# NVIDIAGameWorks/RayTracingDenoiser

Hardware: AMD Instinct MI355X
Metric: Mpixels/s REBLUR_DIFFUSE_SPECULAR @1440p (higher is better)
Workload: dtype f32; 1 GPU; REBLUR_DIFFUSE_SPECULAR 2560x1440, default settings, analytic scene + 1rpp noise, moving camera; parallelism=1 GPU, storage=reference pool formats (fp16 history, R10G10B10A2 normals)

## Files before the change

raytracingdenoiser_amd/csrc/hip/kernels_reblur_history.hip:

```cpp
#include "passes.h"
#include "reblur_device.h"

namespace nrdhip {

constexpr int TILE_X = 32;
constexpr int TILE_Y = 8;

static const char* CheckSupportedHistory(const ReblurCB& c) {
    if (c.gRectOrigin.x != 0 || c.gRectOrigin.y != 0)
        return "internal error: a pass was handed a non-zero rectOrigin";
    if (c.gOrthoMode != 0.0f)
        return "REBLUR: orthographic projection is not supported (SURVEY.md section 8c)";
    return nullptr;
}

static_assert(TILE_X == 32 && TILE_Y == 8, "planes.h LoadBlockTileBytes: a workgroup covers two 16x16 tiles of one tile row");

namespace hf {
constexpr int BORDER = 2;
constexpr int BUF_X = TILE_X + 2 * BORDER;
constexpr int BUF_Y = TILE_Y + 2 * BORDER;
constexpr int BUF_STRIDE = BUF_X + 1;

constexpr int TAPS = 20;
constexpr uint64_t PackTaps(bool rows) {
    uint64_t packed = 0;
    int k = 0;
    for (int j = -2; j <= 2; j++)
        for (int i = -2; i <= 2; i++) {
            if ((i == 0 && j == 0) || ((i < 0 ? -i : i) + (j < 0 ? -j : j) == 4))
                continue;
            packed |= uint64_t((rows ? j : i) + 2) << (3 * k++);
        }
    return packed;
}
constexpr uint64_t TAP_I = PackTaps(false), TAP_J = PackTaps(true);
}

namespace hf {
constexpr int TAP_BATCH = 2;
static_assert(TAP_BATCH > 0 && TAPS % TAP_BATCH == 0, "hf::TAP_BATCH: a divisor of 20");
}

struct HfPlanes {
    Plane tiles, normalRoughness, data1, viewZ, inDiff, inSpec, inDiffFast, inSpecFast, outDiff, outSpec, outDiffFast, outSpecFast;
    Plane inDiffSh, inSpecSh, outDiffSh, outSpecSh;
    NormalRoughnessGuide decodedNR;
};

struct HfPixel {
    int px, py, tx, ty;
    float viewZ, roughness, materialID, frustumSize;
    float3 N, Nv, Xv;
    float2 pixelUv;
};

template <bool IS_SPEC, bool DIFF, bool SPEC, bool PERF, int KIND, bool SH>
NRD_D typename ReblurSignal<KIND>::type HistoryFixSignal(const ReblurCB& c, const HfPlanes& P, const HfPixel& s, typename ReblurSignal<KIND>::type sig, float frameNum, float strideBase,
    const Plane& gIn_Signal, const Plane& gIn_Fast, const Plane& gOut_Fast, const float* s_Luma, float4& sh, const Plane& gIn_Sh) {
    typedef ReblurSignal<KIND> Sig;
    typedef typename Sig::type S;
    const int rw = c.gRectSizeMinusOne.x, rh = c.gRectSizeMinusOne.y;
    const float smc = GetSpecMagicCurve(s.roughness);

    float stride = strideBase * (frameNum < c.gHistoryFixFrameNum ? 1.0f : 0.0f);
    if (IS_SPEC)
        stride *= Lerp(0.5f, 1.0f, smc);
    stride = floorf(stride);

    if (stride != 0.0f) {
        const int stridei = (int)(stride + 0.5f);
        const float nonLinearAccumSpeed = Rcp(1.0f + frameNum);
        const float r = IS_SPEC ? s.roughness : 1.0f;
        const float2 rectSizeInv = ToF2(c.gRectSizeInv);
        const float4 hitDistParams = ToF4(c.gHitDistParams);

        float normalWeightParam = GetNormalWeightParam(nonLinearAccumSpeed, c.gLobeAngleFraction, r);
        float2 geometryWeightParams = GetGeometryWeightParams(c.gPlaneDistSensitivity, s.frustumSize, s.Xv, s.Nv);
        float2 relaxedRoughnessWeightParams = GetRelaxedRoughnessWeightParams(s.roughness * s.roughness, Sqrt(c.gRoughnessFraction));

        float hitDistScale = GetHitDistanceNormalization(s.viewZ, hitDistParams, r);
        float hitDist = ExtractHitDist(sig) * hitDistScale;
        float hitDistFactor = GetHitDistFactor(hitDist, s.frustumSize);
        float2 hitDistanceWeightParams = GetHitDistanceWeightParams(hitDistFactor, nonLinearAccumSpeed, r);

        float sumw = 1.0f + frameNum;
        if (PERF)
            sumw = 1.0f + Rcp(1.0f + c.gMaxAccumulatedFrameNum) - nonLinearAccumSpeed;
        sig = sig * sumw;
        if (SH)
            sh = F4(sh.x * sumw, sh.y * sumw, sh.z * sumw, IS_SPEC ? sh.w : sh.w * sumw);

        const float minMaterial = IS_SPEC ? c.gSpecMinMaterial : c.gDiffMinMaterial;
        const bool compareMaterials = minMaterial < 3.0f;

        const float rcpFrustumSize = Rcp(s.frustumSize);
        const float hitDistEdgeBase = LinearStep(0.03f, 0.05f, s.roughness);
        const float hitDistEdge = 0.2f + hitDistEdgeBase;
        const float hitDistRcpRange = Rcp((0.05f + hitDistEdgeBase) - hitDistEdge);

        struct Tap {
            float4 normalViewZ;
            uint32_t roughnessWord;
            float2 data1;
            S smp;
            float4 sh;
        };
        auto reconstruct = [&](auto materials) {
            constexpr bool MATERIALS = decltype(materials)::value;
            auto requestTap = [&](int i, int j) {
                const int sx = ClampI(s.px + i * stridei, 0, rw), sy = ClampI(s.py + j * stridei, 0, rh);
                Tap t;
                const uint32_t offset = TexelOffset(P.decodedNR.nz, sx, sy, 16u, true);
                t.normalViewZ = *(const float4*)(P.decodedNR.nz.ptr + offset);
                t.roughnessWord = 0u;
                if (IS_SPEC || MATERIALS)
                    t.roughnessWord = *(const uint32_t*)(P.decodedNR.word.ptr + (offset >> 2));
                t.data1 = F2(0.0f, 0.0f);
                if (!PERF)
                    t.data1 = LoadData1<DIFF, SPEC>(P.data1, sx, sy);
                t.smp = Sig::Load(gIn_Signal, sx, sy);
                t.sh = F4(0.0f);
                if (SH)
                    t.sh = LoadRGBA16F(gIn_Sh, sx, sy);
                return t;
            };
            auto addTap = [&](const Tap& t, int i, int j) {
                float2 uv = s.pixelUv + F2(float(i), float(j)) * stride * rectSizeInv;

                float zs = t.normalViewZ.w;
                float4 Ns = F4(t.normalViewZ.x, t.normalViewZ.y, t.normalViewZ.z, DecodedRoughness(t.roughnessWord));

                float angle = AcosApprox(Dot(Xyz(Ns), s.N));
                float3 Xvs = ReconstructViewPosition(uv, ToF4(c.gFrustum), zs, NRD_ORTHO_MODE(c));

                float w = IsInScreenNearest(uv);
                w *= ComputeWeight(Dot(s.Nv, Xvs), geometryWeightParams.x, geometryWeightParams.y);
                if (MATERIALS)
                    w *= CompareMaterials(s.materialID, DecodedMaterialID(t.roughnessWord), minMaterial) ? 1.0f : 0.0f;
                w *= ComputeExponentialWeight(angle, normalWeightParam, 0.0f);
                if (IS_SPEC)
                    w *= ComputeExponentialWeight(Ns.w * Ns.w, relaxedRoughnessWeightParams.x, relaxedRoughnessWeightParams.y);

                if (!PERF)
                    w *= 1.0f + (IS_SPEC ? t.data1.y : t.data1.x);

                S smp = Select(w == 0.0f, Sig::Zero(), t.smp);

                float hs = ExtractHitDist(smp) * hitDistScale;
                float hsFactor = Sat(hs * rcpFrustumSize);
                w *= ComputeExponentialWeight(hsFactor, hitDistanceWeightParams.x, hitDistanceWeightParams.y);

                if (IS_SPEC) {
                    float d = Div(Abs(hitDist - hs), Max(hitDist, hs) + 0.001f);
                    w *= SmoothStep01(Sat((d - hitDistEdge) * hitDistRcpRange));
                }

                sumw += w;
                sig = Mad(smp, w, sig);
                if (SH) {
                    float4 tsh = Select(w == 0.0f, F4(0.0f), t.sh);
                    sh = F4(sh.x + tsh.x * w, sh.y + tsh.y * w, sh.z + tsh.z * w, IS_SPEC ? sh.w : sh.w + tsh.w * w);
                }
            };

#pragma unroll 1
            for (int first = 0; first < hf::TAPS; first += hf::TAP_BATCH) {
                Tap taps[hf::TAP_BATCH];
#pragma unroll
                for (int n = 0; n < hf::TAP_BATCH; n++)
                    taps[n] = requestTap(int((hf::TAP_I >> (3 * (first + n))) & 7u) - 2, int((hf::TAP_J >> (3 * (first + n))) & 7u) - 2);
#pragma unroll
                for (int n = 0; n < hf::TAP_BATCH; n++)
                    addTap(taps[n], int((hf::TAP_I >> (3 * (first + n))) & 7u) - 2, int((hf::TAP_J >> (3 * (first + n))) & 7u) - 2);
            }
        };
        if (compareMaterials)
            reconstruct(std::true_type());
        else
            reconstruct(std::false_type());

        sumw = PositiveRcp(sumw);
        sig = sig * sumw;
        if (SH)
            sh = F4(sh.x * sumw, sh.y * sumw, sh.z * sumw, IS_SPEC ? sh.w : sh.w * sumw);
    }

    float center = s_Luma[(s.ty + hf::BORDER) * hf::BUF_STRIDE + s.tx + hf::BORDER];
    float m1 = center, m2 = center * center;

    float f = Sat(Div(frameNum, c.gHistoryFixFrameNum + NRD_EPS));
    if (IS_SPEC)
        f = Lerp(1.0f, f, smc);
    center = Lerp(GetLuma(sig), center, f);
    Sig::StoreFast(gOut_Fast, s.px, s.py, center);

#pragma unroll
    for (int j = 0; j <= 4; j++) {
#pragma unroll
        for (int i = 0; i <= 4; i++) {
            if (i == 2 && j == 2)
                continue;
            float d = s_Luma[(s.ty + j) * hf::BUF_STRIDE + s.tx + i];
            m1 += d;
            m2 += d * d;
        }
    }

    float luma = GetLuma(sig);

    if (KIND == SIGNAL_RADIANCE && c.gAntiFirefly != 0.0f) {
        float am1 = 0.0f, am2 = 0.0f;
        const int R = PERF ? 3 : REBLUR_ANTI_FIREFLY_FILTER_RADIUS;
        for (int j = -R; j <= R; j++)
            for (int i = -R; i <= R; i++) {
                if (abs(i) <= 1 && abs(j) <= 1)
                    continue;
                float d = LoadR16F(gIn_Fast, ClampI(s.px + i, 0, rw), ClampI(s.py + j, 0, rh));
                am1 += d;
                am2 += d * d;
            }
        float invNorm = Rcp(float((R * 2 + 1) * (R * 2 + 1) - 3 * 3));
        am1 *= invNorm;
        am2 *= invNorm;
        float sigma = Sqrt(Abs(am2 - am1 * am1)) * REBLUR_ANTI_FIREFLY_SIGMA_SCALE;
        luma = Clamp(luma, am1 - sigma, am1 + sigma);
    }

    m1 = m1 * (1.0f / 25.0f);
    m2 = m2 * (1.0f / 25.0f);
    float sigma = Sqrt(Abs(m2 - m1 * m1)) * (KIND != SIGNAL_RADIANCE ? REBLUR_COLOR_CLAMPING_SIGMA_SCALE_OCCLUSION : REBLUR_COLOR_CLAMPING_SIGMA_SCALE);
    float lumaClamped = Clamp(luma, m1 - sigma, m1 + sigma);
    luma = Lerp(lumaClamped, luma, Rcp(1.0f + (c.gMaxFastAccumulatedFrameNum < c.gMaxAccumulatedFrameNum ? 1.0f : 0.0f) * frameNum * 2.0f));

    if (SH) {
        float k = GetLumaScale(Length(Xyz(sh)), luma);
        sh = F4(sh.x * k, sh.y * k, sh.z * k, sh.w);
    }
    return ChangeLuma(sig, luma);
}

template <bool DIFF, bool SPEC, bool PERF, int KIND, bool SH>
__global__ __launch_bounds__(TILE_X* TILE_Y, SH ? 0 : NRD_WAVES_REBLUR_HF - (PERF ? 1 : 0)) void ReblurHistoryFixKernel(ReblurCB c, HfPlanes P, RowRange rr) {
    typedef ReblurSignal<KIND> Sig;
    typedef typename Sig::type S;
    __shared__ float s_DiffLuma[DIFF ? hf::BUF_Y * hf::BUF_STRIDE : 1];
    __shared__ float s_SpecLuma[SPEC ? hf::BUF_Y * hf::BUF_STRIDE : 1];

    const int tx = threadIdx.x % TILE_X, ty = threadIdx.x / TILE_X;
    const int blockY = BlockTileY(rr);
    const int tileX = BlockTileXRotated(rr, blockY);
    const int px = tileX * TILE_X + tx, py = blockY * TILE_Y + ty;
    const int rw = c.gRectSizeMinusOne.x, rh = c.gRectSizeMinusOne.y;

    const uint32_t tileBytes = LoadBlockTileBytes(P.tiles, tileX, blockY);
    if (!TileBytesHaveGeometry<2>(tileBytes))
        return;
    const int qx = min(px, rw), qy = min(max(py, 0), rh);
    const bool preSky = TileByteIsSky(tileBytes, tx >> 4);
    float preMaterialID, preViewZ;
    const float4 preNormalAndRoughness = LoadDecodedNormalRoughness(P.decodedNR, qx, qy, preMaterialID, preViewZ);
    const float2 preData1 = LoadData1<DIFF, SPEC>(P.data1, qx, qy);
    S preDiff = Sig::Zero(), preSpec = Sig::Zero();
    if (DIFF)
        preDiff = Sig::Load(P.inDiff, qx, qy);
    if (SPEC)
        preSpec = Sig::Load(P.inSpec, qx, qy);
    {
        const int baseX = tileX * TILE_X - hf::BORDER, baseY = blockY * TILE_Y - hf::BORDER;
        for (int i = threadIdx.x; i < hf::BUF_X * hf::BUF_Y; i += TILE_X * TILE_Y) {
            int lx = i % hf::BUF_X, ly = i / hf::BUF_X;
            int gx = ClampI(baseX + lx, 0, rw), gy = ClampI(baseY + ly, 0, rh);
            if (DIFF)
                s_DiffLuma[ly * hf::BUF_STRIDE + lx] = Sig::LoadFast(P.inDiffFast, gx, gy);
            if (SPEC)
                s_SpecLuma[ly * hf::BUF_STRIDE + lx] = Sig::LoadFast(P.inSpecFast, gx, gy);
        }
    }
    __syncthreads();

    if (px > rw || py > rh || py < rr.rowBegin || py >= rr.rowEnd)
        return;
    if (preSky)
        return;
    HfPixel s;
    s.viewZ = preViewZ;
    if (s.viewZ > c.gDenoisingRange)
        return;

    s.px = px, s.py = py, s.tx = tx, s.ty = ty;
    s.materialID = preMaterialID;
    float4 normalAndRoughness = preNormalAndRoughness;
    s.N = Xyz(normalAndRoughness);
    s.roughness = normalAndRoughness.w;
    s.frustumSize = GetFrustumSize(c.gMinRectDimMulUnproject, NRD_ORTHO_MODE(c), s.viewZ);
    s.pixelUv = F2(float(px) + 0.5f, float(py) + 0.5f) * ToF2(c.gRectSizeInv);
    s.Xv = ReconstructViewPosition(s.pixelUv, ToF4(c.gFrustum), s.viewZ, NRD_ORTHO_MODE(c));
    s.Nv = RotateVectorInverse(c.gViewToWorld, s.N);
    float2 frameNum = preData1;
    float2 stride = F2(Div(c.gHistoryFixBasePixelStride, 2.0f + frameNum.x), Div(c.gHistoryFixBasePixelStride, 2.0f + frameNum.y));

    if (DIFF) {
        float4 diffSh = F4(0.0f);
        if (SH)
            diffSh = LoadRGBA16F(P.inDiffSh, px, py);
        S diff = HistoryFixSignal<false, DIFF, SPEC, PERF, KIND, SH>(c, P, s, preDiff, frameNum.x, stride.x, P.inDiff, P.inDiffFast, P.outDiffFast, s_DiffLuma, diffSh, P.inDiffSh);
        Sig::Store(P.outDiff, px, py, diff);
        if (SH)
            StoreRGBA16F(P.outDiffSh, px, py, diffSh);
    }
    if (SPEC) {
        float4 specSh = F4(0.0f);
        if (SH)
            specSh = LoadRGBA16F(P.inSpecSh, px, py);
        S spec = HistoryFixSignal<true, DIFF, SPEC, PERF, KIND, SH>(c, P, s, preSpec, frameNum.y, stride.y, P.inSpec, P.inSpecFast, P.outSpecFast, s_SpecLuma, specSh, P.inSpecSh);
        Sig::Store(P.outSpec, px, py, spec);
        if (SH)
            StoreRGBA16F(P.outSpecSh, px, py, specSh);
    }
}

template <bool DIFF, bool SPEC, bool PERF, int KIND, bool SH>
static const char* LaunchHistoryFix(const PassArgs& a) {
    const ReblurCB& c = *(const ReblurCB*)a.constants;
    if (const char* err = CheckSupportedHistory(c))
        return err;
    HfPlanes P = {};
    uint32_t k = 0;
    P.tiles = a.planes[k++];
    P.normalRoughness = a.planes[k++];
    if (const char* err = MakeNormalRoughnessGuide(a, P.decodedNR))
        return err;
    P.data1 = a.planes[k++];
    P.viewZ = a.planes[k++];
    if (DIFF) P.inDiff = a.planes[k++];
    if (SPEC) P.inSpec = a.planes[k++];
    if (DIFF) P.inDiffFast = a.planes[k++];
    if (SPEC) P.inSpecFast = a.planes[k++];
    if (DIFF && SH) P.inDiffSh = a.planes[k++];
    if (SPEC && SH) P.inSpecSh = a.planes[k++];
    if (DIFF) P.outDiff = a.planes[k++];
    if (SPEC) P.outSpec = a.planes[k++];
    if (DIFF) P.outDiffFast = a.planes[k++];
    if (SPEC) P.outSpecFast = a.planes[k++];
    if (DIFF && SH) P.outDiffSh = a.planes[k++];
    if (SPEC && SH) P.outSpecSh = a.planes[k++];
    if (k != a.planesNum)
        return "REBLUR history fix: unexpected resource count";
    RowGrid g = GridForRows(c.gRectSizeMinusOne.x + 1, c.gRectSizeMinusOne.y + 1, TILE_X, TILE_Y, a.rowBegin, a.rowEnd);
    LaunchPass(a, (ReblurHistoryFixKernel<DIFF, SPEC, PERF, KIND, SH>), g.grid, dim3(TILE_X * TILE_Y), c, P, MakeRowRange(g));
    return nullptr;
}

namespace ts {
constexpr int BORDER = 1;
constexpr int BUF_X = TILE_X + 2 * BORDER;
constexpr int BUF_Y = TILE_Y + 2 * BORDER;
constexpr int BUF_STRIDE = BUF_X + 1;
}

struct TsPlanes {
    Plane tiles, normalRoughness, viewZ, data1, data2, inDiff, inSpec, historyDiffLuma, historySpecLuma, inSpecHitDistForTracking, mv, outInternalData, outDiff, outSpec, outDiffLuma,
        outSpecLuma;
    Plane inDiffSh, inSpecSh, outDiffSh, outSpecSh;
    NormalRoughnessGuide decodedNR;
    Plane baseColorMetalness;
};

template <bool PERF>
NRD_D void LumaStats(const ReblurCB& c, const float* s_Luma, int tx, int ty, float& luma, float& m1, float& sigma) {
    luma = s_Luma[(ty + ts::BORDER) * ts::BUF_STRIDE + tx + ts::BORDER];
    float M1 = luma, M2 = luma * luma, mn = NRD_INF, mx = -NRD_INF;
#pragma unroll
    for (int j = 0; j <= 2; j++) {
#pragma unroll
        for (int i = 0; i <= 2; i++) {
            if (i == 1 && j == 1)
                continue;
            float d = s_Luma[(ty + j) * ts::BUF_STRIDE + tx + i];
            M1 += d;
            M2 += d * d;
            mn = Min(mn, d);
            mx = Max(mx, d);
        }
    }
    M1 = M1 * (1.0f / 9.0f);
    M2 = M2 * (1.0f / 9.0f);
    m1 = M1;
    sigma = Sqrt(Abs(M2 - M1 * M1));
    if (!PERF && c.gMaxBlurRadius != 0.0f)
        luma = Clamp(luma, mn, mx);
}

template <bool DIFF, bool SPEC, bool PERF, bool SH, int KIND, bool MVMOD>
__global__ __launch_bounds__(TILE_X* TILE_Y, NRD_WAVES_REBLUR_TS) void ReblurTemporalStabilizationKernel(ReblurCB c, TsPlanes P, RowRange rr) {
    typedef ReblurSignal<KIND> Sig;
    typedef typename Sig::type S;
    __shared__ float s_DiffLuma[DIFF ? ts::BUF_Y * ts::BUF_STRIDE : 1];
    __shared__ float s_SpecLuma[SPEC ? ts::BUF_Y * ts::BUF_STRIDE : 1];

    const int tx = threadIdx.x % TILE_X, ty = threadIdx.x / TILE_X;
    const int blockY = BlockTileY(rr);
    const int px = BlockTileX(rr) * TILE_X + tx, py = blockY * TILE_Y + ty;
    const int rw = c.gRectSizeMinusOne.x, rh = c.gRectSizeMinusOne.y;

    const uint32_t tileBytes = LoadBlockTileBytes(P.tiles, BlockTileX(rr), blockY);
    if (!TileBytesHaveGeometry<2>(tileBytes))
        return;
    const int qx = min(px, rw), qy = min(max(py, 0), rh);
    const bool preSky = TileByteIsSky(tileBytes, tx >> 4);
    const float preViewZ = LoadR32F(P.viewZ, qx, qy);
    const float4 preMv = LoadRGBA16F(P.mv, qx, qy);
    float preMaterialID;
    const float4 preNormalAndRoughness = LoadDecodedNormalRoughness(P.decodedNR, qx, qy, preMaterialID);
    const float2 preData1 = LoadData1<DIFF, SPEC>(P.data1, qx, qy);
    const uint32_t preData2 = SPEC ? LoadR32U(P.data2, qx, qy) : LoadR8U(P.data2, qx, qy);
    S preDiff = Sig::Zero(), preSpec = Sig::Zero();
    if (DIFF)
        preDiff = Sig::Load(P.inDiff, qx, qy);
    if (SPEC)
        preSpec = Sig::Load(P.inSpec, qx, qy);
    {
        const int baseX = BlockTileX(rr) * TILE_X - ts::BORDER, baseY = blockY * TILE_Y - ts::BORDER;
        for (int i = threadIdx.x; i < ts::BUF_X * ts::BUF_Y; i += TILE_X * TILE_Y) {
            int lx = i % ts::BUF_X, ly = i / ts::BUF_X;
            int gx = ClampI(baseX + lx, 0, rw), gy = ClampI(baseY + ly, 0, rh);
            if (DIFF)
                s_DiffLuma[ly * ts::BUF_STRIDE + lx] = GetLuma(Sig::Load(P.inDiff, gx, gy));
            if (SPEC)
                s_SpecLuma[ly * ts::BUF_STRIDE + lx] = GetLuma(Sig::Load(P.inSpec, gx, gy));
        }
    }
    __syncthreads();
// ... 251 lines not shown
```

raytracingdenoiser_amd/csrc/hip/planes.h:

```cpp
#pragma once

#include <hip/hip_fp16.h>
#include <hip/hip_runtime.h>

#include <cstdint>
#include <type_traits>

namespace nrdhip {

struct Plane {
    uint8_t* ptr;
    uint32_t pitch;
    int32_t w, h;
};

#define NRD_D __device__ __forceinline__

NRD_D void ShareLayout(Plane& p, const Plane& ref) {
    p.pitch = ref.pitch;
    p.w = ref.w;
    p.h = ref.h;
}
NRD_D void ShareSize(Plane& p, const Plane& ref) {
    p.w = ref.w;
// ... 33 lines not shown
#define NRD_DIV_15(k) DivSmallIntByConst(k, 15.0f, 0.06666667014360428f)
#define NRD_DIV_3(k) DivSmallIntByConst(k, 3.0f, 0.3333333432674408f)

#ifndef NRD_LDS_WHOLE_TEXEL
#define NRD_LDS_WHOLE_TEXEL(v) asm("" : "+v"(v.x), "+v"(v.y), "+v"(v.z), "+v"(v.w))
#endif
NRD_D float4 LdsFloat4(const float4* p) {
    float4 v = *p;
    NRD_LDS_WHOLE_TEXEL(v);
    return v;
}

NRD_D float HalfBitsToFloat(uint16_t h) { return __half2float(__ushort_as_half(h)); }
#ifndef NRD_OPAQUE_CVT_F16
#define NRD_OPAQUE_CVT_F16(h, f) asm("v_cvt_f16_f32 %0, %1" : "=v"(h) : "v"(f))
#endif
NRD_D uint16_t FloatToHalfBits(float f) {
    uint32_t h;
    NRD_OPAQUE_CVT_F16(h, f);
    return (uint16_t)h;
}

NRD_D float LoadR32F(const Plane& p, int x, int y) { return *TexelPtr<const float>(p, x, y); }
NRD_D void StoreR32F(const Plane& p, int x, int y, float v) { *TexelPtr<float>(p, x, y) = v; }
NRD_D uint32_t LoadR32U(const Plane& p, int x, int y) { return *TexelPtr<const uint32_t>(p, x, y); }
NRD_D void StoreR32U(const Plane& p, int x, int y, uint32_t v) { *TexelPtr<uint32_t>(p, x, y) = v; }
NRD_D uint32_t LoadR16U(const Plane& p, int x, int y) { return *TexelPtr<const uint16_t>(p, x, y); }
NRD_D void StoreR16U(const Plane& p, int x, int y, uint32_t v) { *TexelPtr<uint16_t>(p, x, y) = (uint16_t)v; }
NRD_D uint32_t LoadR8U(const Plane& p, int x, int y) { return *TexelPtr<const uint8_t>(p, x, y); }
NRD_D void StoreR8U(const Plane& p, int x, int y, uint32_t v) { *TexelPtr<uint8_t>(p, x, y) = (uint8_t)v; }

template <int N, int BPT = 1>
NRD_D uint32_t LoadTileBytesUniform(const Plane& tiles, int tileX0, int tileY) {
    static_assert((N == 1 || N == 2 || N == 4) && (BPT == 1 || BPT == 2) && N * BPT <= 4, "the tiles under a workgroup lie in one aligned dword");
    const int cx = min(tileX0, tiles.w - 1), cy = min(tileY, tiles.h - 1);
    uint32_t bytes = 0;
#if defined(__HIP_DEVICE_COMPILE__)
    const uint32_t offset = (uint32_t)__builtin_amdgcn_readfirstlane((int)(__umul24((uint32_t)cy, tiles.pitch) + (((uint32_t)cx * BPT) & ~3u)));
    typedef const uint32_t __attribute__((address_space(4))) ConstDword;
    const uint32_t raw = *(ConstDword*)(uintptr_t)(tiles.ptr + offset) >> ((((uint32_t)cx * BPT) & 3u) * 8u);
    for (int t = 0; t < N; t++)
        bytes |= ((raw >> (8 * BPT * t)) & 0xFFu) << (8 * t);
#else
    for (int t = 0; t < N; t++)
        bytes |= (cx + t < tiles.w ? (uint32_t)tiles.ptr[(uint32_t)cy * tiles.pitch + (uint32_t)(cx + t) * BPT] : 0xFFu) << (8 * t);
#endif
    uint32_t outside = (tileX0 >= tiles.w || tileY >= tiles.h) ? 0xFFFFFFFFu : 0u;
    for (int t = 1; t < N; t++)
        outside |= tileX0 + t >= tiles.w ? 0xFFu << (8 * t) : 0u;
    return (bytes | outside) & (N == 4 ? 0xFFFFFFFFu : (1u << (8 * (N & 3))) - 1u);
}
template <int N>
NRD_D bool TileBytesHaveGeometry(uint32_t bytes) {
    bool any = false;
    for (int t = 0; t < N; t++)
        any |= ((bytes >> (8 * t)) & 0xFFu) == 0u;
    return any;
}
NRD_D bool TileByteIsSky(uint32_t bytes, int t) { return ((bytes >> (8 * t)) & 0xFFu) != 0u; }
NRD_D uint32_t LoadBlockTileBytes(const Plane& tiles, int blockX, int blockY) { return LoadTileBytesUniform<2>(tiles, blockX * 2, blockY >> 1); }

constexpr int TILE_FLAG_GROUP = 64;
NRD_D bool AnyTileFlagUniform(const Plane& flags, int firstTile, int row) {
    const int count = min(flags.w - firstTile, TILE_FLAG_GROUP);
    uint32_t any = 0;
#if defined(__HIP_DEVICE_COMPILE__)
    typedef uint32_t Dwords __attribute__((ext_vector_type(TILE_FLAG_GROUP / 4)));
    typedef const Dwords __attribute__((address_space(4))) ConstDwords;
    const uint32_t offset = (uint32_t)__builtin_amdgcn_readfirstlane((int)(__umul24((uint32_t)row, flags.pitch) + (uint32_t)firstTile));
    const Dwords v = *(ConstDwords*)(uintptr_t)(flags.ptr + offset);
#pragma unroll
    for (int i = 0; i < TILE_FLAG_GROUP / 4; i++) {
        const int n = count - 4 * i;
        any |= n >= 4 ? v[i] : (n > 0 ? v[i] & ((1u << (8 * n)) - 1u) : 0u);
    }
#else
    for (int k = 0; k < count; k++)
        any |= flags.ptr[(uint32_t)row * flags.pitch + (uint32_t)(firstTile + k)];
#endif
    return any != 0u;
}
NRD_D bool TileFlagUniform(const Plane& flags, int tile, int row) { return LoadTileBytesUniform<1>(flags, tile, row) != 0u; }

NRD_D float LoadR16F(const Plane& p, int x, int y) { return HalfBitsToFloat(*TexelPtr<const uint16_t>(p, x, y)); }
NRD_D void StoreR16F(const Plane& p, int x, int y, float v) { *TexelPtr<uint16_t>(p, x, y) = FloatToHalfBits(v); }

NRD_D float4 LoadRGBA16F(const Plane& p, int x, int y) {
    uint2 raw = *TexelPtr<const uint2>(p, x, y);
    float4 r;
    r.x = HalfBitsToFloat((uint16_t)(raw.x & 0xFFFFu));
    r.y = HalfBitsToFloat((uint16_t)(raw.x >> 16));
    r.z = HalfBitsToFloat((uint16_t)(raw.y & 0xFFFFu));
    r.w = HalfBitsToFloat((uint16_t)(raw.y >> 16));
    return r;
}
#ifndef NRD_OPAQUE_CVT_PK_F16
#define NRD_OPAQUE_CVT_PK_F16(r, a, b) asm("v_cvt_pk_f16_f32 %0, %1, %2" : "=v"(r) : "v"(a), "v"(b))
#endif
NRD_D uint32_t FloatsToHalf2Bits(float lo, float hi) {
    uint32_t r;
    NRD_OPAQUE_CVT_PK_F16(r, lo, hi);
    return r;
}
NRD_D void StoreRGBA16F(const Plane& p, int x, int y, float4 v) {
    uint2 raw;
    raw.x = FloatsToHalf2Bits(v.x, v.y);
    raw.y = FloatsToHalf2Bits(v.z, v.w);
    *TexelPtr<uint2>(p, x, y) = raw;
}

#ifndef NRD_NT_STORE_PIXELS
#define NRD_NT_STORE_PIXELS 6000000u
#endif
template <bool NT>
NRD_D void StoreRGBA16FHinted(const Plane& p, int x, int y, float4 v) {
    if constexpr (NT) {
        typedef uint32_t V2 __attribute__((ext_vector_type(2)));
        V2 raw;
        raw.x = FloatsToHalf2Bits(v.x, v.y);
        raw.y = FloatsToHalf2Bits(v.z, v.w);
        __builtin_nontemporal_store(raw, (V2*)TexelPtr<uint2>(p, x, y));
    } else {
        StoreRGBA16F(p, x, y, v);
    }
}

NRD_D float4 LoadRGBA32F(const Plane& p, int x, int y) { return *TexelPtr<const float4>(p, x, y); }
NRD_D void StoreRGBA32F(const Plane& p, int x, int y, float4 v) { *TexelPtr<float4>(p, x, y) = v; }

struct Rgb32Texel {
    float x, y, z;
};
static_assert(sizeof(Rgb32Texel) == 12 && alignof(Rgb32Texel) == 4, "RGB32_SFLOAT texels are three packed dwords");
NRD_D float3 LoadXyz32F(const Plane& p, int x, int y, uint32_t bytesPerTexel) {
    const Rgb32Texel v = *(const Rgb32Texel*)(p.ptr + TexelOffset(p, x, y, bytesPerTexel, true));
    return make_float3(v.x, v.y, v.z);
}
NRD_D float3 LoadRGB32F(const Plane& p, int x, int y) { return LoadXyz32F(p, x, y, 12u); }
NRD_D void StoreRGB32F(const Plane& p, int x, int y, float3 v) { *TexelPtr<Rgb32Texel>(p, x, y) = Rgb32Texel{v.x, v.y, v.z}; }

NRD_D float Saturate(float x) { return fminf(fmaxf(x, 0.0f), 1.0f); }
NRD_D uint32_t ToUnorm(float x, float maxValue) { return (uint32_t)floorf(Saturate(x) * maxValue + 0.5f); }

NRD_D float LoadR8Unorm(const Plane& p, int x, int y) { return NRD_DIV_255(float(*TexelPtr<const uint8_t>(p, x, y))); }
NRD_D void StoreR8Unorm(const Plane& p, int x, int y, float v) { *TexelPtr<uint8_t>(p, x, y) = (uint8_t)ToUnorm(v, 255.0f); }

NRD_D float LoadR16Unorm(const Plane& p, int x, int y) { return NRD_DIV_65535(float(*TexelPtr<const uint16_t>(p, x, y))); }
NRD_D void StoreR16Unorm(const Plane& p, int x, int y, float v) { *TexelPtr<uint16_t>(p, x, y) = (uint16_t)ToUnorm(v, 65535.0f); }

NRD_D float FromSnorm16(uint32_t bits16) { return fmaxf(NRD_DIV_32767(float((int32_t)(int16_t)bits16)), -1.0f); }
NRD_D uint32_t ToSnorm16(float x) {
    float c = fminf(fmaxf(x, -1.0f), 1.0f) * 32767.0f;
    int32_t i = c >= 0.0f ? (int32_t)floorf(c + 0.5f) : -(int32_t)floorf(-c + 0.5f);
    return (uint32_t)i & 0xFFFFu;
}
NRD_D float4 LoadRGBA16Snorm(const Plane& p, int x, int y) {
    uint2 raw = *TexelPtr<const uint2>(p, x, y);
    return make_float4(FromSnorm16(raw.x & 0xFFFFu), FromSnorm16(raw.x >> 16), FromSnorm16(raw.y & 0xFFFFu), FromSnorm16(raw.y >> 16));
}
NRD_D void StoreRGBA16Snorm(const Plane& p, int x, int y, float4 v) {
    uint2 raw;
    raw.x = ToSnorm16(v.x) | (ToSnorm16(v.y) << 16);
    raw.y = ToSnorm16(v.z) | (ToSnorm16(v.w) << 16);
    *TexelPtr<uint2>(p, x, y) = raw;
}

// ... 38 lines not shown
```

Baseline: 5401 Mpixels/s.

## Redistribute history-fix reconstruction taps cooperatively across the workgroup

Adds a cooperative path to the REBLUR history-fix kernel. When only a few pixels in a tile have young history and need the 20-tap reconstruction, their per-pixel parameters are stored in LDS and the (pixel, tap) jobs are spread over all threads, so sparse divergent waves no longer run the full tap loop serially. A cost heuristic (and an env override) decides between the cooperative path and the original per-pixel loop. The cost is extra LDS, extra barriers, ballots and recomputation of per-pixel state, and the path is compiled only when SH is off.

New measurement: 5426 Mpixels/s, median of 6. About the same (+0.5%).

```diff
diff --git a/raytracingdenoiser_amd/csrc/hip/kernels_reblur_history.hip b/raytracingdenoiser_amd/csrc/hip/kernels_reblur_history.hip
--- a/raytracingdenoiser_amd/csrc/hip/kernels_reblur_history.hip
+++ b/raytracingdenoiser_amd/csrc/hip/kernels_reblur_history.hip
@@ -1,5 +1,7 @@
 #include "passes.h"
 #include "reblur_device.h"
+
+#include <cstdio>
 
 namespace nrdhip {
 
@@ -42,6 +44,12 @@
 static_assert(TAP_BATCH > 0 && TAPS % TAP_BATCH == 0, "hf::TAP_BATCH: a divisor of 20");
 }
 
+namespace hf {
+constexpr int MAX_PAIRS = 32;
+constexpr int MAX_JOBS = MAX_PAIRS * TAPS;
+constexpr int KAPPA_NUM = 3, KAPPA_DEN = 2;
+}
+
 struct HfPlanes {
     Plane tiles, normalRoughness, data1, viewZ, inDiff, inSpec, inDiffFast, inSpecFast, outDiff, outSpec, outDiffFast, outSpecFast;
     Plane inDiffSh, inSpecSh, outDiffSh, outSpecSh;
@@ -49,44 +57,191 @@
 };
 
 struct HfPixel {
-    int px, py, tx, ty;
+    int px, py, x0, y0;
     float viewZ, roughness, materialID, frustumSize;
     float3 N, Nv, Xv;
     float2 pixelUv;
 };
 
+struct alignas(16) HfTapParams {
+    int px, py;
+    float stride, materialID;
+    float3 N;
+    float normalWeightParam;
+    float3 Nv;
+    float hitDistScale;
+    float2 pixelUv, geometryWeightParams;
+    float2 relaxedRoughnessWeightParams, hitDistanceWeightParams;
+    float hitDist, rcpFrustumSize, hitDistEdge, hitDistRcpRange;
+};
+static_assert(sizeof(HfTapParams) == 96, "hf::MAX_PAIRS: the LDS budget counts 96 bytes per pair");
+
+template <typename S>
+struct HfTap {
+    float4 normalViewZ;
+    uint32_t roughnessWord;
+    float2 data1;
+    S smp;
+    float4 sh;
+};
+
+template <bool IS_SPEC>
+NRD_D float HistoryFixStride(const ReblurCB& c, float frameNum, float strideBase, float smc) {
+    float stride = strideBase * (frameNum < c.gHistoryFixFrameNum ? 1.0f : 0.0f);
+    if (IS_SPEC)
+        stride *= Lerp(0.5f, 1.0f, smc);
+    return floorf(stride);
+}
+
+template <bool IS_SPEC, typename S>
+NRD_D HfTapParams MakeHfTapParams(const ReblurCB& c, const HfPixel& s, S sig, float frameNum, float stride) {
+    const float nonLinearAccumSpeed = Rcp(1.0f + frameNum);
+    const float r = IS_SPEC ? s.roughness : 1.0f;
+    const float4 hitDistParams = ToF4(c.gHitDistParams);
+
+    HfTapParams t;
+    t.px = s.px, t.py = s.py;
+    t.stride = stride;
+    t.materialID = s.materialID;
+    t.N = s.N, t.Nv = s.Nv;
+    t.pixelUv = s.pixelUv;
+    t.normalWeightParam = GetNormalWeightParam(nonLinearAccumSpeed, c.gLobeAngleFraction, r);
+    t.geometryWeightParams = GetGeometryWeightParams(c.gPlaneDistSensitivity, s.frustumSize, s.Xv, s.Nv);
+    t.relaxedRoughnessWeightParams = F2(0.0f, 0.0f);
+    if (IS_SPEC)
+        t.relaxedRoughnessWeightParams = GetRelaxedRoughnessWeightParams(s.roughness * s.roughness, Sqrt(c.gRoughnessFraction));
+
+    t.hitDistScale = GetHitDistanceNormalization(s.viewZ, hitDistParams, r);
+    t.hitDist = ExtractHitDist(sig) * t.hitDistScale;
+    float hitDistFactor = GetHitDistFactor(t.hitDist, s.frustumSize);
+    t.hitDistanceWeightParams = GetHitDistanceWeightParams(hitDistFactor, nonLinearAccumSpeed, r);
+
+    t.rcpFrustumSize = Rcp(s.frustumSize);
+    t.hitDistEdge = 0.0f, t.hitDistRcpRange = 0.0f;
+    if (IS_SPEC) {
+        const float hitDistEdgeBase = LinearStep(0.03f, 0.05f, s.roughness);
+        t.hitDistEdge = 0.2f + hitDistEdgeBase;
+        t.hitDistRcpRange = Rcp((0.05f + hitDistEdgeBase) - t.hitDistEdge);
+    }
+    return t;
+}
+
+template <bool PERF>
+NRD_D float HfOwnWeight(const ReblurCB& c, float frameNum) {
+    float sumw = 1.0f + frameNum;
+    if (PERF)
+        sumw = 1.0f + Rcp(1.0f + c.gMaxAccumulatedFrameNum) - Rcp(1.0f + frameNum);
+    return sumw;
+}
+
+template <bool IS_SPEC, bool DIFF, bool SPEC, bool PERF, int KIND, bool SH, bool MATERIALS>
+NRD_D HfTap<typename ReblurSignal<KIND>::type> HfRequestTap(const ReblurCB& c, const HfPlanes& P, const HfTapParams& p, const Plane& gIn_Signal, const Plane& gIn_Sh, int i, int j) {
+    typedef ReblurSignal<KIND> Sig;
+    const int rw = c.gRectSizeMinusOne.x, rh = c.gRectSizeMinusOne.y;
+    const int stridei = (int)(p.stride + 0.5f);
+    const int sx = ClampI(p.px + i * stridei, 0, rw), sy = ClampI(p.py + j * stridei, 0, rh);
+    HfTap<typename Sig::type> t;
+    const uint32_t offset = TexelOffset(P.decodedNR.nz, sx, sy, 16u, true);
+    t.normalViewZ = *(const float4*)(P.decodedNR.nz.ptr + offset);
+    t.roughnessWord = 0u;
+    if (IS_SPEC || MATERIALS)
+        t.roughnessWord = *(const uint32_t*)(P.decodedNR.word.ptr + (offset >> 2));
+    t.data1 = F2(0.0f, 0.0f);
+    if (!PERF)
+        t.data1 = LoadData1<DIFF, SPEC>(P.data1, sx, sy);
+    t.smp = Sig::Load(gIn_Signal, sx, sy);
+    t.sh = F4(0.0f);
+    if (SH)
+        t.sh = LoadRGBA16F(gIn_Sh, sx, sy);
+    return t;
+}
+template <bool IS_SPEC, bool PERF, int KIND, bool MATERIALS>
+NRD_D float HfTapWeight(const ReblurCB& c, const HfTapParams& p, float minMaterial, const HfTap<typename ReblurSignal<KIND>::type>& t, int i, int j,
+    typename ReblurSignal<KIND>::type& smp) {
+    const float2 rectSizeInv = ToF2(c.gRectSizeInv);
+    float2 uv = p.pixelUv + F2(float(i), float(j)) * p.stride * rectSizeInv;
+
+    float zs = t.normalViewZ.w;
+    float4 Ns = F4(t.normalViewZ.x, t.normalViewZ.y, t.normalViewZ.z, DecodedRoughness(t.roughnessWord));
+
+    float angle = AcosApprox(Dot(Xyz(Ns), p.N));
+    float3 Xvs = ReconstructViewPosition(uv, ToF4(c.gFrustum), zs, NRD_ORTHO_MODE(c));
+
+    float w = IsInScreenNearest(uv);
+    w *= ComputeWeight(Dot(p.Nv, Xvs), p.geometryWeightParams.x, p.geometryWeightParams.y);
+    if (MATERIALS)
+        w *= CompareMaterials(p.materialID, DecodedMaterialID(t.roughnessWord), minMaterial) ? 1.0f : 0.0f;
+    w *= ComputeExponentialWeight(angle, p.normalWeightParam, 0.0f);
+    if (IS_SPEC)
+        w *= ComputeExponentialWeight(Ns.w * Ns.w, p.relaxedRoughnessWeightParams.x, p.relaxedRoughnessWeightParams.y);
+
+    if (!PERF)
+        w *= 1.0f + (IS_SPEC ? t.data1.y : t.data1.x);
+
+    smp = Select(w == 0.0f, ReblurSignal<KIND>::Zero(), t.smp);
+
+    float hs = ExtractHitDist(smp) * p.hitDistScale;
+    float hsFactor = Sat(hs * p.rcpFrustumSize);
+    w *= ComputeExponentialWeight(hsFactor, p.hitDistanceWeightParams.x, p.hitDistanceWeightParams.y);
+
+    if (IS_SPEC) {
+        float d = Div(Abs(p.hitDist - hs), Max(p.hitDist, hs) + 0.001f);
+        w *= SmoothStep01(Sat((d - p.hitDistEdge) * p.hitDistRcpRange));
+    }
+    return w;
+}
+
+template <bool IS_SPEC, bool DIFF, bool SPEC, bool PERF, int KIND, bool MATERIALS>
+NRD_D void HfCoopTap(const ReblurCB& c, const HfPlanes& P, const Plane& gIn_Signal, float minMaterial, const HfTapParams* s_Rec, int rec, int k, float* s_TapW,
+    typename ReblurSignal<KIND>::type* s_TapSmp, int slot) {
+    const HfTapParams p = s_Rec[rec];
+    const int i = int((hf::TAP_I >> (3 * k)) & 7u) - 2, j = int((hf::TAP_J >> (3 * k)) & 7u) - 2;
+    const auto t = HfRequestTap<IS_SPEC, DIFF, SPEC, PERF, KIND, false, MATERIALS>(c, P, p, gIn_Signal, gIn_Signal, i, j);
+    typename ReblurSignal<KIND>::type smp;
+    const float w = HfTapWeight<IS_SPEC, PERF, KIND, MATERIALS>(c, p, minMaterial, t, i, j, smp);
+    s_TapW[slot] = w;
+    s_TapSmp[slot] = smp;
+}
+template <bool IS_SPEC, bool DIFF, bool SPEC, bool PERF, int KIND>
+NRD_D void HfCoopTaps(const ReblurCB& c, const HfPlanes& P, const Plane& gIn_Signal, const HfTapParams* s_Rec, int firstRec, int count, int first, float* s_TapW,
+    typename ReblurSignal<KIND>::type* s_TapSmp) {
+    const float minMaterial = IS_SPEC ? c.gSpecMinMaterial : c.gDiffMinMaterial;
+    const bool compareMaterials = minMaterial < 3.0f;
+    for (int n = first; n < count * hf::TAPS; n += TILE_X * TILE_Y) {
+        const int pair = n / hf::TAPS, k = n - pair * hf::TAPS;
+        if (compareMaterials)
+            HfCoopTap<IS_SPEC, DIFF, SPEC, PERF, KIND, true>(c, P, gIn_Signal, minMaterial, s_Rec, firstRec + pair, k, s_TapW, s_TapSmp, firstRec * hf::TAPS + n);
+        else
+            HfCoopTap<IS_SPEC, DIFF, SPEC, PERF, KIND, false>(c, P, gIn_Signal, minMaterial, s_Rec, firstRec + pair, k, s_TapW, s_TapSmp, firstRec * hf::TAPS + n);
+    }
+}
+template <bool PERF, typename S>
+NRD_D S HfCoopSum(const ReblurCB& c, S sig, float frameNum, const float* s_TapW, const S* s_TapSmp, int rec) {
+    float sumw = HfOwnWeight<PERF>(c, frameNum);
+    sig = sig * sumw;
+#pragma unroll 4
+    for (int k = 0; k < hf::TAPS; k++) {
+        const float w = s_TapW[rec * hf::TAPS + k];
+        const S smp = s_TapSmp[rec * hf::TAPS + k];
+        sumw += w;
+        sig = Mad(smp, w, sig);
+    }
+    sumw = PositiveRcp(sumw);
+    return sig * sumw;
+}
+
 template <bool IS_SPEC, bool DIFF, bool SPEC, bool PERF, int KIND, bool SH>
-NRD_D typename ReblurSignal<KIND>::type HistoryFixSignal(const ReblurCB& c, const HfPlanes& P, const HfPixel& s, typename ReblurSignal<KIND>::type sig, float frameNum, float strideBase,
-    const Plane& gIn_Signal, const Plane& gIn_Fast, const Plane& gOut_Fast, const float* s_Luma, float4& sh, const Plane& gIn_Sh) {
+NRD_D typename ReblurSignal<KIND>::type HistoryFixSignal(const ReblurCB& c, const HfPlanes& P, const HfPixel& s, typename ReblurSignal<KIND>::type sig, float frameNum, float stride,
+    bool reconstructed, const Plane& gIn_Signal, const Plane& gIn_Fast, const Plane& gOut_Fast, const float* s_Luma, float4& sh, const Plane& gIn_Sh) {
     typedef ReblurSignal<KIND> Sig;
     typedef typename Sig::type S;
     const int rw = c.gRectSizeMinusOne.x, rh = c.gRectSizeMinusOne.y;
     const float smc = GetSpecMagicCurve(s.roughness);
 
-    float stride = strideBase * (frameNum < c.gHistoryFixFrameNum ? 1.0f : 0.0f);
-    if (IS_SPEC)
-        stride *= Lerp(0.5f, 1.0f, smc);
-    stride = floorf(stride);
-
-    if (stride != 0.0f) {
-        const int stridei = (int)(stride + 0.5f);
-        const float nonLinearAccumSpeed = Rcp(1.0f + frameNum);
-        const float r = IS_SPEC ? s.roughness : 1.0f;
-        const float2 rectSizeInv = ToF2(c.gRectSizeInv);
-        const float4 hitDistParams = ToF4(c.gHitDistParams);
-
-        float normalWeightParam = GetNormalWeightParam(nonLinearAccumSpeed, c.gLobeAngleFraction, r);
-        float2 geometryWeightParams = GetGeometryWeightParams(c.gPlaneDistSensitivity, s.frustumSize, s.Xv, s.Nv);
-        float2 relaxedRoughnessWeightParams = GetRelaxedRoughnessWeightParams(s.roughness * s.roughness, Sqrt(c.gRoughnessFraction));
-
-        float hitDistScale = GetHitDistanceNormalization(s.viewZ, hitDistParams, r);
-        float hitDist = ExtractHitDist(sig) * hitDistScale;
-        float hitDistFactor = GetHitDistFactor(hitDist, s.frustumSize);
-        float2 hitDistanceWeightParams = GetHitDistanceWeightParams(hitDistFactor, nonLinearAccumSpeed, r);
-
-        float sumw = 1.0f + frameNum;
-        if (PERF)
-            sumw = 1.0f + Rcp(1.0f + c.gMaxAccumulatedFrameNum) - nonLinearAccumSpeed;
+    if (stride != 0.0f && !reconstructed) {
+        const HfTapParams p = MakeHfTapParams<IS_SPEC>(c, s, sig, frameNum, stride);
+
+        float sumw = HfOwnWeight<PERF>(c, frameNum);
         sig = sig * sumw;
         if (SH)
             sh = F4(sh.x * sumw, sh.y * sumw, sh.z * sumw, IS_SPEC ? sh.w : sh.w * sumw);
@@ -94,68 +249,11 @@
         const float minMaterial = IS_SPEC ? c.gSpecMinMaterial : c.gDiffMinMaterial;
         const bool compareMaterials = minMaterial < 3.0f;
 
-        const float rcpFrustumSize = Rcp(s.frustumSize);
-        const float hitDistEdgeBase = LinearStep(0.03f, 0.05f, s.roughness);
-        const float hitDistEdge = 0.2f + hitDistEdgeBase;
-        const float hitDistRcpRange = Rcp((0.05f + hitDistEdgeBase) - hitDistEdge);
-
-        struct Tap {
-            float4 normalViewZ;
-            uint32_t roughnessWord;
-            float2 data1;
-            S smp;
-            float4 sh;
-        };
         auto reconstruct = [&](auto materials) {
             constexpr bool MATERIALS = decltype(materials)::value;
-            auto requestTap = [&](int i, int j) {
-                const int sx = ClampI(s.px + i * stridei, 0, rw), sy = ClampI(s.py + j * stridei, 0, rh);
-                Tap t;
-                const uint32_t offset = TexelOffset(P.decodedNR.nz, sx, sy, 16u, true);
-                t.normalViewZ = *(const float4*)(P.decodedNR.nz.ptr + offset);
-                t.roughnessWord = 0u;
-                if (IS_SPEC || MATERIALS)
-                    t.roughnessWord = *(const uint32_t*)(P.decodedNR.word.ptr + (offset >> 2));
-                t.data1 = F2(0.0f, 0.0f);
-                if (!PERF)
-                    t.data1 = LoadData1<DIFF, SPEC>(P.data1, sx, sy);
-                t.smp = Sig::Load(gIn_Signal, sx, sy);
-                t.sh = F4(0.0f);
-                if (SH)
-                    t.sh = LoadRGBA16F(gIn_Sh, sx, sy);
-                return t;
-            };
-            auto addTap = [&](const Tap& t, int i, int j) {
-                float2 uv = s.pixelUv + F2(float(i), float(j)) * stride * rectSizeInv;
-
-                float zs = t.normalViewZ.w;
-                float4 Ns = F4(t.normalViewZ.x, t.normalViewZ.y, t.normalViewZ.z, DecodedRoughness(t.roughnessWord));
-
-                float angle = AcosApprox(Dot(Xyz(Ns), s.N));
-                float3 Xvs = ReconstructViewPosition(uv, ToF4(c.gFrustum), zs, NRD_ORTHO_MODE(c));
-
-                float w = IsInScreenNearest(uv);
-                w *= ComputeWeight(Dot(s.Nv, Xvs), geometryWeightParams.x, geometryWeightParams.y);
-                if (MATERIALS)
-                    w *= CompareMaterials(s.materialID, DecodedMaterialID(t.roughnessWord), minMaterial) ? 1.0f : 0.0f;
-                w *= ComputeExponentialWeight(angle, normalWeightParam, 0.0f);
-                if (IS_SPEC)
-                    w *= ComputeExponentialWeight(Ns.w * Ns.w, relaxedRoughnessWeightParams.x, relaxedRoughnessWeightParams.y);
-
-                if (!PERF)
-                    w *= 1.0f + (IS_SPEC ? t.data1.y : t.data1.x);
-
-                S smp = Select(w == 0.0f, Sig::Zero(), t.smp);
-
-                float hs = ExtractHitDist(smp) * hitDistScale;
-                float hsFactor = Sat(hs * rcpFrustumSize);
-                w *= ComputeExponentialWeight(hsFactor, hitDistanceWeightParams.x, hitDistanceWeightParams.y);
-
-                if (IS_SPEC) {
-                    float d = Div(Abs(hitDist - hs), Max(hitDist, hs) + 0.001f);
-                    w *= SmoothStep01(Sat((d - hitDistEdge) * hitDistRcpRange));
-                }
-
+            auto addTap = [&](const HfTap<S>& t, int i, int j) {
+                S smp;
+                const float w = HfTapWeight<IS_SPEC, PERF, KIND, MATERIALS>(c, p, minMaterial, t, i, j, smp);
                 sumw += w;
                 sig = Mad(smp, w, sig);
                 if (SH) {
@@ -166,10 +264,11 @@
 
 #pragma unroll 1
             for (int first = 0; first < hf::TAPS; first += hf::TAP_BATCH) {
-                Tap taps[hf::TAP_BATCH];
+                HfTap<S> taps[hf::TAP_BATCH];
 #pragma unroll
                 for (int n = 0; n < hf::TAP_BATCH; n++)
-                    taps[n] = requestTap(int((hf::TAP_I >> (3 * (first + n))) & 7u) - 2, int((hf::TAP_J >> (3 * (first + n))) & 7u) - 2);
+                    taps[n] = HfRequestTap<IS_SPEC, DIFF, SPEC, PERF, KIND, SH, MATERIALS>(c, P, p, gIn_Signal, gIn_Sh, int((hf::TAP_I >> (3 * (first + n))) & 7u) - 2,
+                        int((hf::TAP_J >> (3 * (first + n))) & 7u) - 2);
 #pragma unroll
                 for (int n = 0; n < hf::TAP_BATCH; n++)
                     addTap(taps[n], int((hf::TAP_I >> (3 * (first + n))) & 7u) - 2, int((hf::TAP_J >> (3 * (first + n))) & 7u) - 2);
@@ -186,7 +285,11 @@
             sh = F4(sh.x * sumw, sh.y * sumw, sh.z * sumw, IS_SPEC ? sh.w : sh.w * sumw);
     }
 
-    float center = s_Luma[(s.ty + hf::BORDER) * hf::BUF_STRIDE + s.tx + hf::BORDER];
+    int tx = s.px, ty = s.py;
+    NRD_OPAQUE_VALUE(tx);
+    NRD_OPAQUE_VALUE(ty);
+    tx -= s.x0, ty -= s.y0;
+    float center = s_Luma[(ty + hf::BORDER) * hf::BUF_STRIDE + tx + hf::BORDER];
     float m1 = center, m2 = center * center;
 
     float f = Sat(Div(frameNum, c.gHistoryFixFrameNum + NRD_EPS));
@@ -201,7 +304,7 @@
         for (int i = 0; i <= 4; i++) {
             if (i == 2 && j == 2)
                 continue;
-            float d = s_Luma[(s.ty + j) * hf::BUF_STRIDE + s.tx + i];
+            float d = s_Luma[(ty + j) * hf::BUF_STRIDE + tx + i];
             m1 += d;
             m2 += d * d;
         }
@@ -241,11 +344,18 @@
 }
 
 template <bool DIFF, bool SPEC, bool PERF, int KIND, bool SH>
-__global__ __launch_bounds__(TILE_X* TILE_Y, SH ? 0 : NRD_WAVES_REBLUR_HF - (PERF ? 1 : 0)) void ReblurHistoryFixKernel(ReblurCB c, HfPlanes P, RowRange rr) {
+__global__ __launch_bounds__(TILE_X* TILE_Y, SH ? 0 : NRD_WAVES_REBLUR_HF - (PERF ? 1 : 0)) void ReblurHistoryFixKernel(ReblurCB c, HfPlanes P, RowRange rr, int coopHook) {
     typedef ReblurSignal<KIND> Sig;
     typedef typename Sig::type S;
+    constexpr bool COOP = !SH;
+    constexpr int WAVES = TILE_X * TILE_Y / 64;
     __shared__ float s_DiffLuma[DIFF ? hf::BUF_Y * hf::BUF_STRIDE : 1];
     __shared__ float s_SpecLuma[SPEC ? hf::BUF_Y * hf::BUF_STRIDE : 1];
+    alignas(16) __shared__ uint32_t s_AnyYoung[WAVES];
+    __shared__ uint64_t s_YoungMask[WAVES][2];
+    __shared__ HfTapParams s_Rec[COOP ? hf::MAX_PAIRS : 1];
+    __shared__ float s_TapW[COOP ? hf::MAX_JOBS : 1];
+    __shared__ S s_TapSmp[COOP ? hf::MAX_JOBS : 1];
 
     const int tx = threadIdx.x % TILE_X, ty = threadIdx.x / TILE_X;
     const int blockY = BlockTileY(rr);
@@ -258,9 +368,36 @@
         return;
     const int qx = min(px, rw), qy = min(max(py, 0), rh);
     const bool preSky = TileByteIsSky(tileBytes, tx >> 4);
-    float preMaterialID, preViewZ;
-    const float4 preNormalAndRoughness = LoadDecodedNormalRoughness(P.decodedNR, qx, qy, preMaterialID, preViewZ);
-    const float2 preData1 = LoadData1<DIFF, SPEC>(P.data1, qx, qy);
+    struct Own {
+        float4 normalAndRoughness;
+        float materialID, viewZ;
+        float2 frameNum;
+    };
+    auto loadOwn = [&]() {
+        Own o;
+        o.normalAndRoughness = LoadDecodedNormalRoughness(P.decodedNR, qx, qy, o.materialID, o.viewZ);
+        o.frameNum = LoadData1<DIFF, SPEC>(P.data1, qx, qy);
+        return o;
+    };
+    auto strides = [&](const Own& o) {
+        const float2 strideBase = F2(Div(c.gHistoryFixBasePixelStride, 2.0f + o.frameNum.x), Div(c.gHistoryFixBasePixelStride, 2.0f + o.frameNum.y));
+        const float smc = GetSpecMagicCurve(o.normalAndRoughness.w);
+        return F2(HistoryFixStride<false>(c, o.frameNum.x, strideBase.x, smc), HistoryFixStride<true>(c, o.frameNum.y, strideBase.y, smc));
+    };
+    auto makePixel = [&](const Own& o) {
+        HfPixel s;
+        s.viewZ = o.viewZ;
+        s.px = px, s.py = py, s.x0 = tileX * TILE_X, s.y0 = blockY * TILE_Y;
+        s.materialID = o.materialID;
+        s.N = Xyz(o.normalAndRoughness);
+        s.roughness = o.normalAndRoughness.w;
+        s.frustumSize = GetFrustumSize(c.gMinRectDimMulUnproject, NRD_ORTHO_MODE(c), s.viewZ);
+        s.pixelUv = F2(float(px) + 0.5f, float(py) + 0.5f) * ToF2(c.gRectSizeInv);
+        s.Xv = ReconstructViewPosition(s.pixelUv, ToF4(c.gFrustum), s.viewZ, NRD_ORTHO_MODE(c));
+        s.Nv = RotateVectorInverse(c.gViewToWorld, s.N);
+        return s;
+    };
+    Own own = loadOwn();
     S preDiff = Sig::Zero(), preSpec = Sig::Zero();
     if (DIFF)
         preDiff = Sig::Load(P.inDiff, qx, qy);
@@ -277,34 +414,85 @@
                 s_SpecLuma[ly * hf::BUF_STRIDE + lx] = Sig::LoadFast(P.inSpecFast, gx, gy);
         }
     }
+    const bool denoised = !(px > rw || py > rh || py < rr.rowBegin || py >= rr.rowEnd) && !preSky && !(own.viewZ > c.gDenoisingRange);
+    const uint32_t lane = threadIdx.x & 63u, wave = threadIdx.x >> 6;
+    if constexpr (COOP) {
+        const bool maybeYoung = denoised && ((DIFF && own.frameNum.x < c.gHistoryFixFrameNum) || (SPEC && own.frameNum.y < c.gHistoryFixFrameNum));
+        const int any = __any(maybeYoung ? 1 : 0);
+        if (lane == 0u)
+            s_AnyYoung[wave] = any ? 1u : 0u;
+    }
     __syncthreads();
 
-    if (px > rw || py > rh || py < rr.rowBegin || py >= rr.rowEnd)
+    bool coop = false, youngDiff = false, youngSpec = false;
+    int pairsDiff = 0, pairsSpec = 0, pairDiff = 0, pairSpec = 0;
+    static_assert(WAVES == 4, "s_AnyYoung is read as four dwords");
+    if (COOP && (s_AnyYoung[0] | s_AnyYoung[1] | s_AnyYoung[2] | s_AnyYoung[3]) != 0u) {
+        const float2 exact = strides(own);
+        youngDiff = DIFF && denoised && exact.x != 0.0f, youngSpec = SPEC && denoised && exact.y != 0.0f;
+        const uint64_t maskDiff = WaveBallot(youngDiff), maskSpec = WaveBallot(youngSpec);
+        if (lane == 0u)
+            s_YoungMask[wave][0] = maskDiff, s_YoungMask[wave][1] = maskSpec;
+        __syncthreads();
+        int wavesYoung = 0;
+#pragma unroll
+        for (uint32_t w = 0; w < (uint32_t)WAVES; w++) {
+            const uint64_t d = WaveUniform(s_YoungMask[w][0]), sp = WaveUniform(s_YoungMask[w][1]);
+            const uint64_t below = w < wave ? ~0ull : (w == wave ? (1ull << lane) - 1ull : 0ull);
+            pairDiff += CountBits64(d & below), pairSpec += CountBits64(sp & below);
+            pairsDiff += CountBits64(d), pairsSpec += CountBits64(sp);
+            wavesYoung += (d != 0ull ? 1 : 0) + (sp != 0ull ? 1 : 0);
+        }
+        pairSpec += pairsDiff;
+        if (wavesYoung != 0) {
+            const int loopCost = hf::TAPS * wavesYoung, coopCost = (hf::TAPS * pairsDiff + 63) / 64 + (hf::TAPS * pairsSpec + 63) / 64;
+            coop = coopHook < 0 ? hf::KAPPA_NUM * coopCost < hf::KAPPA_DEN * loopCost : coopHook > 0;
+        }
+    }
+
+    if (!coop && !denoised)
         return;
-    if (preSky)
-        return;
-    HfPixel s;
-    s.viewZ = preViewZ;
-    if (s.viewZ > c.gDenoisingRange)
-        return;
-
-    s.px = px, s.py = py, s.tx = tx, s.ty = ty;
-    s.materialID = preMaterialID;
-    float4 normalAndRoughness = preNormalAndRoughness;
-    s.N = Xyz(normalAndRoughness);
-    s.roughness = normalAndRoughness.w;
-    s.frustumSize = GetFrustumSize(c.gMinRectDimMulUnproject, NRD_ORTHO_MODE(c), s.viewZ);
-    s.pixelUv = F2(float(px) + 0.5f, float(py) + 0.5f) * ToF2(c.gRectSizeInv);
-    s.Xv = ReconstructViewPosition(s.pixelUv, ToF4(c.gFrustum), s.viewZ, NRD_ORTHO_MODE(c));
-    s.Nv = RotateVectorInverse(c.gViewToWorld, s.N);
-    float2 frameNum = preData1;
-    float2 stride = F2(Div(c.gHistoryFixBasePixelStride, 2.0f + frameNum.x), Div(c.gHistoryFixBasePixelStride, 2.0f + frameNum.y));
+
+    if (COOP && coop) {
+        const int pairs = pairsDiff + pairsSpec;
+        const int chunk = coopHook > 0 ? min(coopHook, hf::MAX_PAIRS) : hf::MAX_PAIRS;
+        for (int base = 0; base < pairs; base += chunk) {
+            const int n = min(chunk, pairs - base);
+            const int nDiff = min(max(pairsDiff - base, 0), n);
+            const bool ownsDiff = youngDiff && pairDiff >= base && pairDiff < base + n, ownsSpec = youngSpec && pairSpec >= base && pairSpec < base + n;
+            if (DIFF && ownsDiff) {
+                const Own o = loadOwn();
+                s_Rec[pairDiff - base] = MakeHfTapParams<false>(c, makePixel(o), preDiff, o.frameNum.x, strides(o).x);
+            }
+            if (SPEC && ownsSpec) {
+                const Own o = loadOwn();
+                s_Rec[pairSpec - base] = MakeHfTapParams<true>(c, makePixel(o), preSpec, o.frameNum.y, strides(o).y);
+            }
+            __syncthreads();
+            if (DIFF)
+                HfCoopTaps<false, DIFF, SPEC, PERF, KIND>(c, P, P.inDiff, s_Rec, 0, nDiff, (int)threadIdx.x, s_TapW, s_TapSmp);
+            if (SPEC)
+                HfCoopTaps<true, DIFF, SPEC, PERF, KIND>(c, P, P.inSpec, s_Rec, nDiff, n - nDiff, TILE_X * TILE_Y - 1 - (int)threadIdx.x, s_TapW, s_TapSmp);
+            __syncthreads();
+            if (DIFF && ownsDiff)
+                preDiff = HfCoopSum<PERF>(c, preDiff, loadOwn().frameNum.x, s_TapW, s_TapSmp, pairDiff - base);
+            if (SPEC && ownsSpec)
+                preSpec = HfCoopSum<PERF>(c, preSpec, loadOwn().frameNum.y, s_TapW, s_TapSmp, pairSpec - base);
+        }
+        if (!denoised)
+            return;
+        own = loadOwn();
+    }
+    const HfPixel s = makePixel(own);
+    const float2 frameNum = own.frameNum;
+    const float2 stride = strides(own);
+    const float strideDiff = stride.x, strideSpec = stride.y;
 
     if (DIFF) {
         float4 diffSh = F4(0.0f);
         if (SH)
             diffSh = LoadRGBA16F(P.inDiffSh, px, py);
-        S diff = HistoryFixSignal<false, DIFF, SPEC, PERF, KIND, SH>(c, P, s, preDiff, frameNum.x, stride.x, P.inDiff, P.inDiffFast, P.outDiffFast, s_DiffLuma, diffSh, P.inDiffSh);
+        S diff = HistoryFixSignal<false, DIFF, SPEC, PERF, KIND, SH>(c, P, s, preDiff, frameNum.x, strideDiff, coop, P.inDiff, P.inDiffFast, P.outDiffFast, s_DiffLuma, diffSh, P.inDiffSh);
         Sig::Store(P.outDiff, px, py, diff);
         if (SH)
             StoreRGBA16F(P.outDiffSh, px, py, diffSh);
@@ -313,7 +501,7 @@
         float4 specSh = F4(0.0f);
         if (SH)
             specSh = LoadRGBA16F(P.inSpecSh, px, py);
-        S spec = HistoryFixSignal<true, DIFF, SPEC, PERF, KIND, SH>(c, P, s, preSpec, frameNum.y, stride.y, P.inSpec, P.inSpecFast, P.outSpecFast, s_SpecLuma, specSh, P.inSpecSh);
+        S spec = HistoryFixSignal<true, DIFF, SPEC, PERF, KIND, SH>(c, P, s, preSpec, frameNum.y, strideSpec, coop, P.inSpec, P.inSpecFast, P.outSpecFast, s_SpecLuma, specSh, P.inSpecSh);
         Sig::Store(P.outSpec, px, py, spec);
         if (SH)
             StoreRGBA16F(P.outSpecSh, px, py, specSh);
@@ -348,7 +536,11 @@
     if (k != a.planesNum)
         return "REBLUR history fix: unexpected resource count";
     RowGrid g = GridForRows(c.gRectSizeMinusOne.x + 1, c.gRectSizeMinusOne.y + 1, TILE_X, TILE_Y, a.rowBegin, a.rowEnd);
-    LaunchPass(a, (ReblurHistoryFixKernel<DIFF, SPEC, PERF, KIND, SH>), g.grid, dim3(TILE_X * TILE_Y), c, P, MakeRowRange(g));
+    static const char* coopEnv = getenv("NRD_HIP_HF_COOP");
+    int coopHook = -1;
+    if (coopEnv && (sscanf(coopEnv, "%d", &coopHook) != 1 || coopHook < 0))
+        coopHook = -1;
+    LaunchPass(a, (ReblurHistoryFixKernel<DIFF, SPEC, PERF, KIND, SH>), g.grid, dim3(TILE_X * TILE_Y), c, P, MakeRowRange(g), coopHook);
     return nullptr;
 }
 
diff --git a/raytracingdenoiser_amd/csrc/hip/planes.h b/raytracingdenoiser_amd/csrc/hip/planes.h
--- a/raytracingdenoiser_amd/csrc/hip/planes.h
+++ b/raytracingdenoiser_amd/csrc/hip/planes.h
@@ -139,6 +139,28 @@
 }
 NRD_D bool TileFlagUniform(const Plane& flags, int tile, int row) { return LoadTileBytesUniform<1>(flags, tile, row) != 0u; }
 
+NRD_D uint64_t WaveBallot(bool p) {
+#ifdef NRD_EMU
+    const uint32_t lane = threadIdx.x & 63u;
+    uint32_t lo = p && lane < 32u ? 1u << lane : 0u, hi = p && lane >= 32u ? 1u << (lane - 32u) : 0u;
+    for (int o = 1; o < 64; o <<= 1) {
+        lo |= __shfl_xor(lo, o);
+        hi |= __shfl_xor(hi, o);
+    }
+    return (uint64_t)lo | ((uint64_t)hi << 32);
+#else
+    return (uint64_t)__ballot(p ? 1 : 0);
+#endif
+}
+NRD_D int CountBits64(uint64_t m) { return __builtin_popcountll(m); }
+NRD_D uint64_t WaveUniform(uint64_t v) {
+#if defined(__HIP_DEVICE_COMPILE__)
+    return (uint64_t)(uint32_t)__builtin_amdgcn_readfirstlane((int)(uint32_t)v) | ((uint64_t)(uint32_t)__builtin_amdgcn_readfirstlane((int)(uint32_t)(v >> 32)) << 32);
+#else
+    return v;
+#endif
+}
+
 NRD_D float LoadR16F(const Plane& p, int x, int y) { return HalfBitsToFloat(*TexelPtr<const uint16_t>(p, x, y)); }
 NRD_D void StoreR16F(const Plane& p, int x, int y, float v) { *TexelPtr<uint16_t>(p, x, y) = FloatToHalfBits(v); }
 
```
